# Zhengjun-Du/LC-CRF-SLAM

Measured on AMD Instinct MI355X. Metric: CRF mean-field iters/sec, higher is better.
Workload: dtype f32

## Files before the change

lc-crf-slam_amd/csrc/frame_build.h:

```cpp
#pragma once

#include "engine.h"
#include "device_math.h"
#include "fused_loop.h"

namespace lccrf {
namespace fb {

using namespace fl;

constexpr unsigned kEmptyKey = 0x80008000u;
constexpr int kHdr = 512;

struct FrameArgs {
    const float *feat[kMaxFusedK];
    float w[kMaxFusedK];
    float scale[2], inv_dp1, alpha;
    int maxN;
    const int16_t *label;
    float tbl[5];
    int n_iter, with_map;
    float relax;
    int hcap;
    int lds_total;
// ... 38 lines not shown
    const int lane = tid & 63, wave = tid >> 6;
    const int incl = wave_incl_scan(x);
    __syncthreads();
    if (lane == 63) wave_sum[wave] = incl;
    __syncthreads();
    const int ws = lane < NT / 64 ? wave_sum[lane] : 0;
    const int wincl = wave_incl_scan(ws);
    total = __builtin_amdgcn_readlane(wincl, NT / 64 - 1);
    const int wbase = __builtin_amdgcn_readlane(wincl - ws, __builtin_amdgcn_readfirstlane(wave));
    return wbase + incl - x;
}

__device__ __forceinline__ unsigned corner_key(const int16_t (&r0)[2], const uint8_t (&rk)[2], int rem)
{
    const unsigned x = (unsigned short)vertex_coord<2>(r0[0], rk[0], rem);
    const unsigned y = (unsigned short)vertex_coord<2>(r0[1], rk[1], rem);
    return x | (y << 16);
}


template <class T>
__device__ __forceinline__ const T &late_args(int offset)
{
    typedef const __attribute__((address_space(4))) unsigned char *kptr;
    kptr p = (kptr)__builtin_amdgcn_kernarg_segment_ptr();
    asm volatile("" : "+s"(p));
    return *(const T *)(p + offset);
}
constexpr int kArgOffA = (int)((sizeof(CrfDev) + alignof(FrameArgs) - 1) / alignof(FrameArgs) * alignof(FrameArgs));
static_assert(alignof(CrfDev) == 8 && alignof(FrameArgs) == 8, "the frame kernels' arguments (CrfDev, FrameArgs) as the ABI lays them out: by value, naturally aligned, in order");

constexpr int kGridMaxCells = 32768;

__device__ __forceinline__ int wave_min(int x)
{
    x = min(x, __builtin_amdgcn_update_dpp(x, x, 0x111, 0xf, 0xf, false));
    x = min(x, __builtin_amdgcn_update_dpp(x, x, 0x112, 0xf, 0xf, false));
    x = min(x, __builtin_amdgcn_update_dpp(x, x, 0x114, 0xf, 0xf, false));
    x = min(x, __builtin_amdgcn_update_dpp(x, x, 0x118, 0xf, 0xf, false));
    x = min(x, __builtin_amdgcn_update_dpp(x, x, 0x142, 0xa, 0xf, false));
    x = min(x, __builtin_amdgcn_update_dpp(x, x, 0x143, 0xc, 0xf, false));
    return x;
}

struct GridPlace {
    int row;
    int scratch_a;
    int scratch_b;
};
template <int NT, int PPT, class EmitBary>
__device__ __forceinline__ void grid_records(int tid, int N, const float2 (&ftv)[PPT], const float *scale, float inv_dp1, EmitBary emit_bary,
                                             unsigned (&pw)[PPT], unsigned (&pf)[PPT], int *box, int *fail)
{
    constexpr int D1 = kD1;
    const int Npad = (N + 3) & ~3;
    int umin = 0x7fffffff, umax = -0x7fffffff, vmin = 0x7fffffff, vmax = -0x7fffffff;
    bool bad = false;
#pragma unroll
    for (int s = 0; s < PPT; ++s) {
        const int i = tid + s * NT;
        const float2 ft = ftv[s];
        float feat[2] = {i < N ? ft.x : 0.0f, i < N ? ft.y : 0.0f};
        float b[D1];
        int r0x, r0y;
        point_record2_grid(feat, scale, inv_dp1, b, r0x, r0y, pf[s], bad);
        emit_bary(s, i, b);
        const int u = (r0x - r0y) / 3;
        if (i < Npad) {
            umin = min(umin, u); umax = max(umax, u);
            vmin = min(vmin, r0y); vmax = max(vmax, r0y);
        }
        pw[s] = ((unsigned)u & 0xffffu) | ((unsigned)r0y << 16);
    }
    const int lo_u = wave_min(umin), hi_u = wave_min(-umax), lo_v = wave_min(vmin), hi_v = wave_min(-vmax);
    if ((tid & 63) == 63) {
        atomicMin(&box[0], lo_u);
        atomicMin(&box[1], hi_u);
        atomicMin(&box[2], lo_v);
        atomicMin(&box[3], hi_v);
    }
    if (bad) *fail = 1;
}

template <int NT, int PPT, class Place, class StoreNbr>
__device__ __forceinline__ bool grid_build(unsigned char *smem, int tid, int N, const unsigned (&pw)[PPT], const unsigned (&pf)[PPT],
                                           const int *box, const int *fail, int *wave_sum, int floor_lo, int limit, Place place,
                                           StoreNbr store_nbr, int &V_out, unsigned (&pk)[PPT][kD1], int *rowmax, Instr &ins)
{
    constexpr int D1 = kD1;
    const int Npad = (N + 3) & ~3;
    unsigned cell[PPT][D1];
    const int u0 = __builtin_amdgcn_readfirstlane(box[0]) - 2, v0 = __builtin_amdgcn_readfirstlane(box[2]) - 4;
    const int Wp = -__builtin_amdgcn_readfirstlane(box[1]) - u0 + 3, Hp = -__builtin_amdgcn_readfirstlane(box[3]) - v0 + 5;
    const long cells_l = (long)Wp * Hp;
    if (__builtin_amdgcn_readfirstlane(*fail) || cells_l > kGridMaxCells) return false;
    const int cells = (int)cells_l, chunks = (cells + 7) >> 3;
    const int idmap_off = limit - chunks * 16;
    unsigned short *idmap = reinterpret_cast<unsigned short *>(smem + idmap_off);
    if (idmap_off < floor_lo + 64) return false;
    for (int u = tid; u < chunks; u += NT) reinterpret_cast<uint4 *>(idmap)[u] = make_uint4(0u, 0u, 0u, 0u);
    __syncthreads();
#pragma unroll
    for (int s = 0; s < PPT; ++s) {
        const int u = (int)(short)(pw[s] & 0xffffu), v = (int)pw[s] >> 16;
        const int c0 = (u - u0) * Hp + (v - v0);
        cell[s][0] = (unsigned)c0;
        cell[s][1] = (unsigned)(c0 + 1 + ((pf[s] & 4u) ? Hp - 3 : 0) - ((pf[s] & 1u) ? Hp : 0));
        cell[s][2] = (unsigned)(c0 + 2 + ((pf[s] & 8u) ? Hp - 3 : 0) - ((pf[s] & 2u) ? Hp : 0));
#pragma unroll
        for (int j = 0; j < D1; ++j)
            if (tid + s * NT < Npad) idmap[cell[s][j]] = (unsigned short)1;
    }
    __syncthreads();
    FL_PSTAMP();

    const int cpl = (chunks + NT - 1) / NT, c0 = tid * cpl;
    int mine = 0;
    for (int q = 0; q < cpl; ++q) {
        if (c0 + q < chunks) {
            const uint4 w = reinterpret_cast<const uint4 *>(idmap)[c0 + q];
            mine += __popc(w.x) + __popc(w.y) + __popc(w.z) + __popc(w.w);
        }
    }
    int Vk;
    int id = block_excl_scan<NT>(mine, tid, wave_sum, Vk);
    V_out = Vk;
    FL_PSTAMP();
    GridPlace gp;
    if (!place(Vk, gp)) return false;
    auto take = [&](int &o, int bytes) { const int r = o; o += (bytes + 15) & ~15; return r; };
    int vs = gp.scratch_a;
    const int vcell_off = take(vs, Vk * 2);
    const int cnt_off = take(vs, (Vk + 1) * 4);
    const int vs_d = vs;
    vs = max(vs, gp.scratch_b);
    const int E = N * D1;
    const int W = (((Npad + 31) >> 5) + 3) & ~3;
    const bool bitmap = (long)E >= 16L * Vk && vs + 5 * Vk * W + 64 <= limit;
    const int bm_off = vs, pre_off = bm_off + Vk * W * 4;
    const int list_cap = (E + 7 * Vk + 8) & ~7;
    const int list_off = vs;
    const int vs_end = bitmap ? pre_off + Vk * W / 2 : list_off + list_cap * 2;
    if (vs_d > idmap_off || vs_end > limit || Vk >= 32767 || E + 7 * Vk >= 65535) return false;
    unsigned short *vcell = reinterpret_cast<unsigned short *>(smem + vcell_off);
    unsigned *cnt = reinterpret_cast<unsigned *>(smem + cnt_off);
    unsigned *bm = reinterpret_cast<unsigned *>(smem + bm_off);
    unsigned short *pre = reinterpret_cast<unsigned short *>(smem + pre_off);
    unsigned short *list = reinterpret_cast<unsigned short *>(smem + list_off);
    for (int q = 0; q < cpl; ++q) {
        if (c0 + q < chunks) {
            uint4 w = reinterpret_cast<const uint4 *>(idmap)[c0 + q];
            unsigned h[8] = {w.x & 0xffffu, w.x >> 16, w.y & 0xffffu, w.y >> 16, w.z & 0xffffu, w.z >> 16, w.w & 0xffffu, w.w >> 16};
#pragma unroll
            for (int e = 0; e < 8; ++e) {
                if (h[e]) {
                    vcell[id] = (unsigned short)((c0 + q) * 8 + e);
                    h[e] = (unsigned)++id;
                }
            }
            w = make_uint4(h[0] | h[1] << 16, h[2] | h[3] << 16, h[4] | h[5] << 16, h[6] | h[7] << 16);
            reinterpret_cast<uint4 *>(idmap)[c0 + q] = w;
        }
    }
    for (int v = tid; v <= Vk; v += NT) cnt[v] = 0u;
    __syncthreads();
    FL_PSTAMP();

    unsigned vid[PPT][D1], arr[PPT][D1];
#pragma unroll
    for (int s = 0; s < PPT; ++s)
#pragma unroll
        for (int j = 0; j < D1; ++j) vid[s][j] = (tid + s * NT < Npad) ? (unsigned)idmap[cell[s][j]] - 1u : 0u;
#pragma unroll
    for (int s = 0; s < PPT; ++s) {
#pragma unroll
        for (int j = 0; j < D1; ++j) {
            arr[s][j] = 0u;
            if (!bitmap && tid + s * NT < N) arr[s][j] = atomicAdd(&cnt[vid[s][j]], 1u);
        }
    }
    {
        for (int t = tid; t < D1 * Vk; t += NT) {
            const int j = t >= 2 * Vk ? 2 : (t >= Vk ? 1 : 0), v = t - j * Vk;
            const int c = vcell[v], dj = j == 0 ? 1 - Hp : (j == 1 ? Hp - 2 : 1);
            store_nbr(j, v, t, (unsigned)idmap[c - dj] | ((unsigned)idmap[c + dj] << 16));
        }
    }
    __syncthreads();
    FL_PSTAMP();
    if (bitmap) {
        uint4 *b4 = reinterpret_cast<uint4 *>(bm);
        for (int u = tid; u < Vk * W / 4; u += NT) b4[u] = make_uint4(0u, 0u, 0u, 0u);
        __syncthreads();
#pragma unroll
        for (int s = 0; s < PPT; ++s) {
            const int i = tid + s * NT;
            if (i < N) {
#pragma unroll
                for (int j = 0; j < D1; ++j) atomicOr(&bm[vid[s][j] * W + (i >> 5)], 1u << (i & 31));
            }
        }
        __syncthreads();
    } else {
        uint4 *l4 = reinterpret_cast<uint4 *>(list);
        for (int u = tid; u < list_cap / 8; u += NT) l4[u] = make_uint4(0x7fff7fffu, 0x7fff7fffu, 0x7fff7fffu, 0x7fff7fffu);
    }
    FL_PSTAMP();

    if (bitmap) {
        const int lane16 = tid & 15, ng = W >> 2, gpl = (ng + 15) >> 4;
        for (int v = tid >> 4; v < Vk; v += NT / 16) {
            int pc[2] = {0, 0}, sum = 0;
#pragma unroll
            for (int u = 0; u < 2; ++u) {
                const int g = lane16 * gpl + u;
                if (u < gpl && g < ng) {
                    const uint4 b = *reinterpret_cast<const uint4 *>(bm + v * W + 4 * g);
                    pc[u] = __popc(b.x) + __popc(b.y) + __popc(b.z) + __popc(b.w);
                }
                sum += pc[u];
            }
            int incl = sum;
            incl += __builtin_amdgcn_update_dpp(0, incl, 0x111, 0xf, 0xf, false);
            incl += __builtin_amdgcn_update_dpp(0, incl, 0x112, 0xf, 0xf, false);
            incl += __builtin_amdgcn_update_dpp(0, incl, 0x114, 0xf, 0xf, false);
            incl += __builtin_amdgcn_update_dpp(0, incl, 0x118, 0xf, 0xf, false);
            int run = incl - sum;
#pragma unroll
            for (int u = 0; u < 2; ++u) {
                const int g = lane16 * gpl + u;
                if (u < gpl && g < ng) pre[v * ng + g] = (unsigned short)run;
                run += pc[u];
            }
            if (lane16 == 15) cnt[v] = (unsigned)incl;
        }
        __syncthreads();
    }
    unsigned short *row = reinterpret_cast<unsigned short *>(smem + gp.row);
    {
        const int vper = (Vk + 1 + NT - 1) / NT, v0 = tid * vper;
        unsigned sum = 0u;
        int mx = 0;
        for (int u = 0; u < vper; ++u) {
            const int v = v0 + u;
            if (v < Vk) {
                const unsigned n = cnt[v];
                sum += n | (((n + 7u) & ~7u) << 16);
                mx = max(mx, (int)n);
            }
        }
        int tot;
        unsigned run = (unsigned)block_excl_scan<NT>((int)sum, tid, wave_sum, tot);
        for (int u = 0; u < vper; ++u) {
            const int v = v0 + u;
            if (v <= Vk) {
                const unsigned n = v < Vk ? cnt[v] : 0u;
                row[v] = (unsigned short)(run & 0xffffu);
                cnt[v] = (run >> 16) | (n << 16);
                run += n | (((n + 7u) & ~7u) << 16);
            }
        }
        if (rowmax) {
#pragma unroll
            for (int o = 32; o > 0; o >>= 1) mx = max(mx, __shfl_xor(mx, o, 64));
            if ((tid & 63) == 0 && mx > 0) atomicMax(rowmax, mx);
        }
    }
    __syncthreads();
    FL_PSTAMP();

    if (!bitmap) {
#pragma unroll
        for (int s = 0; s < PPT; ++s) {
            const int i = tid + s * NT;
            if (i < N) {
#pragma unroll
                for (int j = 0; j < D1; ++j) list[(cnt[vid[s][j]] & 0xffffu) + arr[s][j]] = (unsigned short)(i * D1 + j);
            }
        }
        __syncthreads();
    }
    FL_PSTAMP();
    auto below = [](const uint4 &x, unsigned e) {
        const unsigned e2 = e | (e << 16), hi = 0x80008000u;
        return 8u - (unsigned)(__popc(((x.x | hi) - e2) & hi) + __popc(((x.y | hi) - e2) & hi) + __popc(((x.z | hi) - e2) & hi) +
                               __popc(((x.w | hi) - e2) & hi));
    };
#pragma unroll
    for (int s = 0; s < PPT; ++s) {
        const int i = tid + s * NT, ic = min(i, N - 1);
        const bool real = i < N;
#pragma unroll
        for (int j = 0; j < D1; ++j) {
            const unsigned v = vid[s][j];
            unsigned r;
            if (bitmap) {
                const uint4 bq = *reinterpret_cast<const uint4 *>(bm + v * W + ((ic >> 5) & ~3));
                const int wq = (ic >> 5) & 3;
                const unsigned low = (1u << (ic & 31)) - 1u;
                r = pre[v * (W >> 2) + (ic >> 7)] + (wq > 0 ? __popc(bq.x) : 0) + (wq > 1 ? __popc(bq.y) : 0) + (wq > 2 ? __popc(bq.z) : 0) +
                    __popc((wq == 0 ? bq.x : wq == 1 ? bq.y : wq == 2 ? bq.z : bq.w) & low);
            } else {
                const unsigned lcv = cnt[v], e = (unsigned)(i * D1 + j);
                const uint4 *lp = reinterpret_cast<const uint4 *>(list + (lcv & 0xffffu));
                r = below(lp[0], e);
                const int n8 = (int)(((lcv >> 16) + 7u) >> 3);
                for (int u = 1; u < n8; ++u) r += below(lp[u], e);
            }
            pk[s][j] = (v + 1u) | (((unsigned)row[v] + (real ? r : 0u)) << 16);
        }
    }
    FL_PSTAMP();
    __syncthreads();
    return true;
}

bool frame_lean_plausible(int NA, int K, int F);
void launch_frame_lean(const CrfDev &c, const FrameArgs &a, int NA, hipStream_t s);

}
}
```

lc-crf-slam_amd/csrc/frame_lean.hip:

```cpp
#include "frame_build.h"
#include "fused_lean.h"

#include <algorithm>
#include <type_traits>

namespace lccrf {
namespace fb {

namespace {

struct LeanHdr {
    int wave_sum[16];
    int fail;
    int box[2][4];
};
constexpr int kLeanHdrBytes = 128;
static_assert(sizeof(LeanHdr) <= kLeanHdrBytes, "header");
template <int PPT>
__global__ void __launch_bounds__(kNTSmall, 4) k_frame_lean(CrfDev c, FrameArgs a)
{
    constexpr int NT = kNTSmall, K = 2, D1 = kD1;
    constexpr bool RELOAD = PPT >= 3;
    extern __shared__ __attribute__((aligned(16))) unsigned char smem[];
    const int f = blockIdx.x, tid = threadIdx.x;
// ... 21 lines not shown
    }
    constexpr int kLds = (int)kLdsHalf;
    constexpr int hdr_off = kLds - kLeanHdrBytes;
    LeanHdr *hdr = reinterpret_cast<LeanHdr *>(smem + hdr_off);

    unsigned char *rec = a.rec + (size_t)f * kLeanRecBytes;
    PointRegs<PPT, K> pr;
    {
        int lab[PPT];
        float2 unr[PPT];
#pragma unroll
        for (int s = 0; s < PPT; ++s) {
            const int ic = min(tid + s * NT, N - 1);
            lab[s] = 0;
            unr[s] = make_float2(0.f, 0.f);
            if (a.label) lab[s] = a.label[(size_t)f * a.maxN + ic];
            else unr[s] = reinterpret_cast<const float2 *>(c.unary)[(size_t)f * c.maxN + ic];
        }
#pragma unroll
        for (int s = 0; s < PPT; ++s) {
            const int i = tid + s * NT;
            float2 un = unr[s];
            if (a.label) {
                const int t = lab[s];
                const bool known = t >= 0 && t < 2;
                un.x = !known ? a.tbl[0] : (t == 0 ? a.tbl[3] : a.tbl[2]);
                un.y = !known ? a.tbl[0] : (t == 1 ? a.tbl[4] : a.tbl[1]);
            }
            if (!RELOAD) pr.un[s] = un;
            else if (i < N) reinterpret_cast<float2 *>(rec + kLeanRecUnary)[i] = un;
        }
    }
    if (tid < 32) reinterpret_cast<float *>(smem)[tid] = 0.0f;
    if (tid < 8) hdr->box[tid >> 2][tid & 3] = 0x7fffffff;
    if (tid == 0) hdr->fail = 0;
    __syncthreads();

    size_t plan = 128;
    int V[K];
    unsigned pk[PPT][K][D1];

    unsigned pw[K][PPT], pf[K][PPT];
    {
        float2 ftv[K][PPT];
#pragma unroll
        for (int k = 0; k < K; ++k)
#pragma unroll
            for (int s = 0; s < PPT; ++s) ftv[k][s] = reinterpret_cast<const float2 *>(a.feat[k])[(size_t)f * a.maxN + min(tid + s * NT, N - 1)];
#pragma unroll
        for (int k = 0; k < K; ++k) {
            auto emit_bary = [&](int s, int i, const float (&b)[D1]) {
                if (!RELOAD) {
#pragma unroll
                    for (int j = 0; j < D1; ++j) pr.bary[s][k][j] = b[j];
                } else if (i < N) {
                    float *bo = reinterpret_cast<float *>(rec + kLeanRecBary + k * (kLeanRecPoints * D1 * 4)) + i * D1;
#pragma unroll
                    for (int j = 0; j < D1; ++j) bo[j] = b[j];
                }
            };
            grid_records<NT, PPT>(tid, N, ftv[k], a.scale, a.inv_dp1, emit_bary, pw[k], pf[k], hdr->box[k], &hdr->fail);
        }
    }
    __syncthreads();
    FL_PSTAMP();
    auto build = [&](auto kc) -> bool {
        constexpr int k = decltype(kc)::value;
        const int plan_before = (int)plan;
        int lt_nbr = 0;
        auto place = [&](int Vk, GridPlace &gp) -> bool {
            if (Vk > lean_max_v(NT) || (k == 0 && (Vk > chain_max_v(NT) || Vk > 256))) return false;
            const LeanTables lt = lean_tables(plan, Vk, k == 0);
            lt_nbr = lt.nbr;
            gp.row = lt.row;
            gp.scratch_a = k == 0 ? (int)plan : plan_before;
            gp.scratch_b = (int)plan;
            return true;
        };
        auto store_nbr = [&](int j, int v, int t, unsigned word) {
            if (k == 0) reinterpret_cast<unsigned *>(smem + lt_nbr)[t] = word;
            else reinterpret_cast<unsigned *>(rec + kLeanRecNbr)[j * (kLeanRecNbrAxis / 4) + v] = word;
        };
        unsigned pkk[PPT][D1];
        const bool ok = grid_build<NT, PPT>(smem, tid, N, pw[k], pf[k], hdr->box[k], &hdr->fail, hdr->wave_sum, plan_before, hdr_off, place,
                                            store_nbr, V[k], pkk, nullptr, ins);
#pragma unroll
        for (int s = 0; s < PPT; ++s)
#pragma unroll
            for (int j = 0; j < D1; ++j) pk[s][k][j] = pkk[s][j];
        return ok;
    };
    if (!build(std::integral_constant<int, 0>{}) || !build(std::integral_constant<int, 1>{})) {
        flag_unfit();
        return;
    }
    FL_STAMP();

    FusedLayout lay;
#pragma unroll
    for (int k = 0; k < K; ++k) V[k] = __builtin_amdgcn_readfirstlane(V[k]);
    {
        if (!layout_lean(N, K, V, kChainMinRow, &lay, NT, (size_t)kLds) || !lay.chain0) {
            flag_unfit();
            return;
        }
    }
    if (tid == 0) {
#pragma unroll
        for (int k = 0; k < K; ++k) {
            reinterpret_cast<float2 *>(smem + lay.val[k][0])[0] = make_float2(0.f, 0.f);
            reinterpret_cast<float2 *>(smem + lay.val[k][1])[0] = make_float2(0.f, 0.f);
        }
    }
    const FrameArgs &al = late_args<FrameArgs>(kArgOffA);
    const CrfDev &cl_ = late_args<CrfDev>(0);
    float wk[K], alpha[K];
    LeanSrc src;
    const __amdgpu_buffer_rsrc_t rsrc = lean_rsrc(rec, kLeanRecBytes);
#pragma unroll
    for (int k = 0; k < K; ++k) {
        wk[k] = al.w[k];
        alpha[k] = al.alpha;
        src.nbr[k] = src.bary[k] = src.norm[k] = rsrc;
        src.off_nbr[k] = kLeanRecNbr;
        src.off_bary[k] = kLeanRecBary + k * (kLeanRecPoints * D1 * 4);
        src.off_norm[k] = kLeanRecNorm + k * (kLeanRecPoints * 4);
        src.nbr_axis_bytes[k] = kLeanRecNbrAxis;
    }
    src.unary = rsrc;
    src.off_unary = kLeanRecUnary;
    __syncthreads();

    ChainLane cl = chain_setup_lean<NT>(smem, lay, V[0], tid);
    place_products_lean<PPT, K, 1, NT>(smem, lay, N, tid, pk, pr);
    FL_STAMP();

#pragma unroll
    for (int s = 0; s < PPT; ++s) pr.q[s] = make_float2(1.0f, 1.0f);
    int t = lane_id();
    mean_field_lean<PPT, K, 1, NT, RELOAD, true>(smem, lay, V, N, t, pr, cl, alpha, wk, src, 1, 0.0f, 0.0f, ins);
    __syncthreads();
    FL_STAMP();

    t = lane_id();
    if (RELOAD) {
#pragma unroll
        for (int s = 0; s < PPT; ++s) {
            typedef unsigned lean_u2 __attribute__((ext_vector_type(2)));
            const lean_u2 u = __builtin_amdgcn_raw_buffer_load_b64(src.unary, (t + s * NT) * 8, src.off_unary, 0);
            pr.un[s] = make_float2(__uint_as_float(u.x), __uint_as_float(u.y));
        }
    }
    start_inference<PPT, K, NT>(pr, N, t);
    mean_field_lean<PPT, K, 1, NT, RELOAD, false>(smem, lay, V, N, t, pr, cl, alpha, wk, src, al.n_iter, al.relax, al.omr, ins);
    t = lane_id();
    store_results<PPT, K, NT>(cl_, f, N, t, pr, al.with_map);
    if (t < K && al.V_out[t]) al.V_out[t][f] = t == 0 ? V[0] : V[K - 1];
    if (t == 0 && al.frame_status) al.frame_status[f] = 0;
    FL_STAMP();
    if (kInstr && al.timing && (int)blockIdx.x == al.timing_block && t == al.timing_lane) al.timing[63] = ins.n;
}

template <int PPT>
void launch_lean_ppt(const CrfDev &c, const FrameArgs &a, hipStream_t s)
{
    auto fn = k_frame_lean<PPT>;
    (void)hipFuncSetAttribute(reinterpret_cast<const void *>(fn), hipFuncAttributeMaxDynamicSharedMemorySize, (int)kLdsLimit);
// ... 24 lines not shown
```

lc-crf-slam_amd/csrc/fused_lean.h:

```cpp
#pragma once

#include "fused_loop.h"

#ifndef LCCRF_LEAN_SKIP
#define LCCRF_LEAN_SKIP 0
#endif
#define LEAN_SKIP(bit) ((LCCRF_LEAN_SKIP & (bit)) != 0)

namespace lccrf {
namespace fl {

constexpr int kLeanMaxRounds = 4;
__host__ __device__ constexpr int lean_rounds(int nt) { return nt >= 512 ? 3 : 4; }
__host__ __device__ constexpr int lean_max_v(int nt) { return 3 * (nt - 64); }

__host__ __device__ inline int lean_plane_floats(int NA, int V0)
{
    const int top = V0 < kChainTop ? V0 : kChainTop;
    return (NA * kD1 + 11 * top + 3 * (V0 - top) + 16 + 63) & ~63;
}

__host__ __device__ inline bool lean_chain_wanted(int NA, int V0, int row0, int nt)
{
    return row0 >= kChainMinRow && V0 <= chain_max_v(nt) && V0 <= 256 && lean_plane_floats(NA, V0) < 65535;
// ... 36 lines not shown
            L.val[k][0] = lt.val0;
            L.val[k][1] = lt.val1;
            L.nbr[k] = lt.nbr;
            L.row[k] = lt.row;
            const size_t pb = (size_t)L.Ecap[k] * 2 * sizeof(float);
            shared_prod = pb > shared_prod ? pb : shared_prod;
        }
        if (o > 65535) return false;
        L.pstart = chain0 ? take((size_t)(V[0] + 2) * sizeof(unsigned short)) : 0;
        const int p = take(shared_prod < 1024 ? 1024 : shared_prod);
        for (int k = 0; k < K; ++k) L.prod[k] = p;
        L.total = (int)o;
        if (o <= lds_limit) {
            *lay = L;
            return true;
        }
    }
    return false;
}

#define LCCRF_ASM_SEL(off, vlo, vhi, S)                                                                             \
    "v_cmp_lt_i32_e32 vcc, " #off ", %[rem]\n\tv_cndmask_b32_e32 %[" #S "], 0, %[ad], vcc\n\t"                     \
    "ds_read_b128 v[" #vlo ":" #vhi "], %[" #S "] offset:" #off "\n\t"

__device__ __forceinline__ float chain_rows_sel(unsigned addr, int bytes, unsigned trips, unsigned &keep0, unsigned &keep1)
{
    float acc = 0.0f;
    if (trips == 0) return acc;
    unsigned sa, sb;
    asm volatile(
        LCCRF_ASM_SEL(0, 96, 99, sa) LCCRF_ASM_SEL(16, 100, 103, sb)
        LCCRF_ASM_SEL(32, 104, 107, sa) LCCRF_ASM_SEL(48, 108, 111, sb)
        LCCRF_ASM_SEL(64, 112, 115, sa) LCCRF_ASM_SEL(80, 116, 119, sb)
        "1:\n\t"
        LCCRF_ASM_SEL(96, 120, 123, sa) LCCRF_ASM_SEL(112, 124, 127, sb)
        "s_waitcnt lgkmcnt(6)\n\t"
        LCCRF_ASM_ADD8(v96, v97, v98, v99, v100, v101, v102, v103)
        "v_add_u32_e32 %[ad], 0x80, %[ad]\n\t"
        "v_subrev_u32_e32 %[rem], 0x80, %[rem]\n\t"
        LCCRF_ASM_SEL(0, 96, 99, sa) LCCRF_ASM_SEL(16, 100, 103, sb)
        "s_waitcnt lgkmcnt(6)\n\t"
        LCCRF_ASM_ADD8(v104, v105, v106, v107, v108, v109, v110, v111)
        LCCRF_ASM_SEL(32, 104, 107, sa) LCCRF_ASM_SEL(48, 108, 111, sb)
        "s_waitcnt lgkmcnt(6)\n\t"
        LCCRF_ASM_ADD8(v112, v113, v114, v115, v116, v117, v118, v119)
        LCCRF_ASM_SEL(64, 112, 115, sa) LCCRF_ASM_SEL(80, 116, 119, sb)
        "s_waitcnt lgkmcnt(6)\n\t"
        LCCRF_ASM_ADD8(v120, v121, v122, v123, v124, v125, v126, v127)
        "s_sub_u32 %[n], %[n], 1\n\t"
        "s_cmp_lg_u32 %[n], 0\n\t"
        "s_cbranch_scc1 1b\n\t"
        "s_waitcnt lgkmcnt(0)\n\t"
        : [acc] "+v"(acc), [ad] "+v"(addr), [rem] "+v"(bytes), [n] "+s"(trips), [sa] "=&v"(sa), [sb] "=&v"(sb), "+v"(keep0), "+v"(keep1)
        :
        : "scc", "vcc", "memory", LCCRF_CHAIN_RING_CLOBBERS);
    return acc;
}

__device__ __forceinline__ float chain_rows_keep(unsigned addr, unsigned end, unsigned trips, unsigned &keep0, unsigned &keep1)
{
    float acc = 0.0f;
    if (trips == 0) return acc;
    const unsigned e1 = end - 32u, e2 = end - 64u, e3 = end - 96u;
    unsigned sel;
    asm volatile(LCCRF_CHAIN_ROWS_ASM
                 : [acc] "+v"(acc), [ad] "+v"(addr), [n] "+s"(trips), [sel] "=&v"(sel), "+v"(keep0), "+v"(keep1)
                 : [e0] "v"(end), [e1] "v"(e1), [e2] "v"(e2), [e3] "v"(e3)
                 : "scc", "memory", LCCRF_CHAIN_RING_CLOBBERS);
    return acc;
}

__device__ __forceinline__ float2 lds_f2(unsigned addr)
{
#if defined(__HIP_DEVICE_COMPILE__)
    typedef float lean_f2 __attribute__((ext_vector_type(2)));
    const lean_f2 v = *reinterpret_cast<const __attribute__((address_space(3))) lean_f2 *>((unsigned long)addr);
    return make_float2(v.x, v.y);
#else
    (void)addr;
    return make_float2(0.f, 0.f);
#endif
}

__device__ __forceinline__ void lds_store_f(unsigned addr, float v)
{
#if defined(__HIP_DEVICE_COMPILE__)
    *reinterpret_cast<__attribute__((address_space(3))) float *>((unsigned long)addr) = v;
#else
    (void)addr; (void)v;
#endif
}
__device__ __forceinline__ void lds_store_f2(unsigned addr, float a, float b)
{
#if defined(__HIP_DEVICE_COMPILE__)
    typedef float lean_f2 __attribute__((ext_vector_type(2)));
    lean_f2 v;
    v.x = a;
    v.y = b;
    *reinterpret_cast<__attribute__((address_space(3))) lean_f2 *>((unsigned long)addr) = v;
#else
    (void)addr; (void)a; (void)b;
#endif
}

template <int PPT, int K, int CH>
__device__ __forceinline__ void point_products_lean(const FusedLayout &lay, const PointRegs<PPT, K> &pr, int s, int k)
{
    const unsigned a0 = (pr.ix[s][k][1] >> 16) << 2, a1 = (pr.ix[s][k][2] & 0xffffu) << 2, a2 = (pr.ix[s][k][2] >> 16) << 2;
    if (chain_k<CH>(lay, k)) {
        const unsigned pb = (unsigned)lay.Ecap[k] * 4u;
        lds_store_f(a0, pr.bary[s][k][0] * pr.q[s].x);
        lds_store_f(a0 + pb, pr.bary[s][k][0] * pr.q[s].y);
        lds_store_f(a1, pr.bary[s][k][1] * pr.q[s].x);
        lds_store_f(a1 + pb, pr.bary[s][k][1] * pr.q[s].y);
        lds_store_f(a2, pr.bary[s][k][2] * pr.q[s].x);
        lds_store_f(a2 + pb, pr.bary[s][k][2] * pr.q[s].y);
    } else {
        lds_store_f2(a0, pr.bary[s][k][0] * pr.q[s].x, pr.bary[s][k][0] * pr.q[s].y);
        lds_store_f2(a1, pr.bary[s][k][1] * pr.q[s].x, pr.bary[s][k][1] * pr.q[s].y);
        lds_store_f2(a2, pr.bary[s][k][2] * pr.q[s].x, pr.bary[s][k][2] * pr.q[s].y);
    }
}

template <int PPT, int K>
__device__ __forceinline__ float2 slice_point_lean(const PointRegs<PPT, K> &pr, int s, int k, float alpha)
{
    const float2 x0 = lds_f2(pr.ix[s][k][0] & 0xffffu), x1 = lds_f2(pr.ix[s][k][0] >> 16), x2 = lds_f2(pr.ix[s][k][1] & 0xffffu);
    const float w0 = pr.bary[s][k][0] * alpha, w1 = pr.bary[s][k][1] * alpha, w2 = pr.bary[s][k][2] * alpha;
    float t0 = w0 * x0.x, t1 = w0 * x0.y;
    t0 += w1 * x1.x; t1 += w1 * x1.y;
    t0 += w2 * x2.x; t1 += w2 * x2.y;
    return make_float2(t0, t1);
}

template <int NT>
__device__ __forceinline__ ChainLane chain_setup_lean(unsigned char *smem, const FusedLayout &lay, int V0, int tid)
{
    constexpr int k = 0;
    ChainLane cl{0u, 0u};
    int *hist = reinterpret_cast<int *>(smem + lay.prod[k]);
    if (tid < 128) hist[tid] = 0;
    __syncthreads();
    const unsigned short *row = reinterpret_cast<const unsigned short *>(smem + lay.row[k]);
    unsigned short *srt = reinterpret_cast<unsigned short *>(smem + lay.prod[k]) + 256;
    unsigned short *pstart = reinterpret_cast<unsigned short *>(smem + lay.pstart);
    int key = 0;
    if (tid < V0) {
        const int len = (int)row[tid + 1] - (int)row[tid];
        key = 63 - min((len + 3) >> 4, 63);
        atomicAdd(&hist[key], 1);
    }
    __syncthreads();
    if (tid < 64) {
        const int x = hist[tid];
        int incl = x;
#pragma unroll
        for (int o = 1; o < 64; o <<= 1) {
            const int y = __shfl_up(incl, o, 64);
            if (tid >= o) incl += y;
        }
        hist[64 + tid] = incl - x;
    }
    __syncthreads();
    if (tid < V0) srt[atomicAdd(&hist[64 + key], 1)] = (unsigned short)tid;
    __syncthreads();
    if (tid < 64) {
        int sz[4], sum = 0;
#pragma unroll
        for (int u = 0; u < 4; ++u) {
            const int r = tid * 4 + u;
            sz[u] = 0;
            if (r < V0) {
                const int v = srt[r];
                const int rl = (int)row[v + 1] - (int)row[v];
                sz[u] = ((rl + 3) & ~3) + (r < kChainTop ? 8 : 0);
            }
            sum += sz[u];
        }
        int incl = sum;
#pragma unroll
        for (int o = 1; o < 64; o <<= 1) {
            const int y = __shfl_up(incl, o, 64);
            if (tid >= o) incl += y;
        }
        int base = incl - sum;
#pragma unroll
        for (int u = 0; u < 4; ++u) {
            const int r = tid * 4 + u;
            if (r < V0) pstart[srt[r]] = (unsigned short)base;
            base += sz[u];
        }
    }
    __syncthreads();
    const int l = (tid >> 6) & 1, pr = tid >> 7, ln = tid & 63;
    const int r = pr == 0 ? (chain_top_rank(ln) >= 0 ? chain_top_rank(ln) : V0) : kChainTop + ((pr - 1) << 6) + ln;
    unsigned quads = 0, addr = 0;
    if (r < V0) {
        const int v = srt[r];
        const int rl = (int)row[v + 1] - (int)row[v], len4 = (rl + 3) & ~3;
        addr = (unsigned)(lay.prod[k] + 4 * (l * lay.Ecap[k] + (int)pstart[v]));
        quads = (unsigned)(len4 >> 2);
        cl.b = quads | ((unsigned)(len4 - rl) << 13) | ((unsigned)((v + 1) * 2 + l) << 16);
    }
    unsigned m = quads;
#pragma unroll
    for (int o = 32; o > 0; o >>= 1) m = max(m, (unsigned)__shfl_xor((int)m, o));
    cl.a = addr | (m << 18);
    __syncthreads();
    return cl;
}

__device__ __forceinline__ void chain_pads_lean(unsigned char *smem, const ChainLane &cl, int tid)
{
    if (cl.b >> 16) {
        float *e = reinterpret_cast<float *>(smem + (cl.a & 0x3ffffu)) + (cl.b & 0x1fffu) * 4u;
        const unsigned npad = (cl.b >> 13) & 3u;
        for (unsigned z = 1; z <= npad; ++z) e[-(int)z] = 0.0f;
        if ((tid >> 7) == 0) {
            reinterpret_cast<float4 *>(e)[0] = make_float4(0.f, 0.f, 0.f, 0.f);
            reinterpret_cast<float4 *>(e)[1] = make_float4(0.f, 0.f, 0.f, 0.f);
        }
    }
}

template <int PPT, int K, int CH, int NT>
__device__ __forceinline__ void place_products_lean(unsigned char *smem, const FusedLayout &lay, int N, int tid,
                                                    const unsigned (&pk)[PPT][K][kD1], PointRegs<PPT, K> &pr)
{
#pragma unroll
    for (int k = 0; k < K; ++k) {
        const unsigned short *row = reinterpret_cast<const unsigned short *>(smem + lay.row[k]);
        const unsigned short *pstart = reinterpret_cast<const unsigned short *>(smem + lay.pstart);
#pragma unroll
        for (int s = 0; s < PPT; ++s) {
            const unsigned vb = (unsigned)lay.val[k][kD1 & 1];
            pr.ix[s][k][0] = (vb + 8u * (pk[s][k][0] & 0xffffu)) | ((vb + 8u * (pk[s][k][1] & 0xffffu)) << 16);
            pr.ix[s][k][1] = vb + 8u * (pk[s][k][2] & 0xffffu);
            pr.ix[s][k][2] = 0;
            if (tid + s * NT < N) {
                unsigned sl[kD1];
#pragma unroll
                for (int j = 0; j < kD1; ++j) {
                    sl[j] = pk[s][k][j] >> 16;
                    if (chain_k<CH>(lay, k)) {
                        const int v = (int)(pk[s][k][j] & 0xffffu) - 1;
                        sl[j] = (unsigned)((int)pstart[v] + ((int)(pk[s][k][j] >> 16) - (int)row[v]));
                        sl[j] = ((unsigned)lay.prod[k] >> 2) + sl[j];
                    } else {
                        sl[j] = ((unsigned)lay.prod[k] >> 2) + 2u * sl[j];
                    }
                }
                pr.ix[s][k][1] |= sl[0] << 16;
                pr.ix[s][k][2] = sl[1] | (sl[2] << 16);
            }
        }
    }
}

typedef unsigned lean_u3 __attribute__((ext_vector_type(3)));
struct LeanSrc {
    __amdgpu_buffer_rsrc_t nbr[kMaxFusedK];
    __amdgpu_buffer_rsrc_t bary[kMaxFusedK];
    __amdgpu_buffer_rsrc_t norm[kMaxFusedK];
    __amdgpu_buffer_rsrc_t unary;
    int nbr_axis_bytes[kMaxFusedK];
    int off_nbr[kMaxFusedK], off_bary[kMaxFusedK], off_norm[kMaxFusedK], off_unary;
};
constexpr int kLeanRecPoints = 4 * kNTSmall;
constexpr int kLeanRecUnary = 0;
constexpr int kLeanRecBary = kLeanRecUnary + kLeanRecPoints * 8;
constexpr int kLeanRecNorm = kLeanRecBary + kMaxFusedK * kLeanRecPoints * kD1 * 4;
constexpr int kLeanRecNbr = kLeanRecNorm + kMaxFusedK * kLeanRecPoints * 4;
constexpr int kLeanRecNbrAxis = lean_max_v(kNTSmall) * 4;
constexpr int kLeanRecBytes = (kLeanRecNbr + kD1 * kLeanRecNbrAxis + 255) & ~255;
__device__ __forceinline__ __amdgpu_buffer_rsrc_t lean_rsrc(const void *p, size_t bytes)
{
    return __builtin_amdgcn_make_buffer_rsrc(const_cast<void *>(p), 0, (int)bytes, 0x00020000);
}

template <int PPT, int K>
__device__ __forceinline__ void opaque_ids(PointRegs<PPT, K> &pr)
{
#pragma unroll
    for (int s = 0; s < PPT; ++s) {
#pragma unroll
        for (int k = 0; k < K; ++k) asm volatile("" : "+v"(pr.ix[s][k][0]), "+v"(pr.ix[s][k][1]), "+v"(pr.ix[s][k][2]));
    }
}

struct LeanPrepPlan {
    int cl_off;
    int row_off[kMaxFusedK], row_bytes[kMaxFusedK];
    int nbr_off[kMaxFusedK], nbr_bytes[kMaxFusedK];
    int total;
};
__host__ __device__ inline LeanPrepPlan lean_prep_plan(const FusedLayout &lay, int K, const int *Vcap, int nt, int ppt)
{
    LeanPrepPlan p{};
    int o = K * ppt * nt * 12;
    p.cl_off = o;
    o += nt * 8;
    for (int k = 0; k < K; ++k) {
        p.row_off[k] = o;
        p.row_bytes[k] = ((Vcap[k] + 2) * 2 + 15) & ~15;
        o += p.row_bytes[k];
        p.nbr_off[k] = o;
        p.nbr_bytes[k] = lay.nbr[k] >= 0 ? ((kD1 * Vcap[k] * 4 + 15) & ~15) : 0;
        o += p.nbr_bytes[k];
    }
    p.total = (o + 255) & ~255;
    return p;
}

template <int PPT, int K, int CH, int NT, bool RELOAD, bool NORM = false, bool PRELOADED = false>
__device__ __forceinline__ void mean_field_lean(unsigned char *smem, const FusedLayout &lay, const int (&V)[K], int N, int &t,
                                                PointRegs<PPT, K> &pr, ChainLane &cl, const float (&alpha)[K],
                                                const float (&wk)[K], const LeanSrc &src, int n_iter, float relax, float omr, Instr &ins)
{
    constexpr int D1 = kD1;
    constexpr int KF = K - 1;
    const int wave_base = __builtin_amdgcn_readfirstlane(t & ~63);
    (void)wave_base;
#define LEAN_FRESH_T()                                                                                               \
    do {                                                                                                             \
        int z_ = 0;                                                                                                  \
        asm volatile("" : "+v"(z_));                                                                                 \
        t = wave_base + (int)__builtin_amdgcn_mbcnt_hi(~0u, __builtin_amdgcn_mbcnt_lo(~0u, (unsigned)z_));          \
    } while (0)
    auto load_weights = [&]() {
        if (!RELOAD) return;
#pragma unroll
        for (int s = 0; s < PPT; ++s) {
            const int i = t + s * NT;
            if (!NORM) {
                typedef unsigned lean_u2 __attribute__((ext_vector_type(2)));
                const lean_u2 u = __builtin_amdgcn_raw_buffer_load_b64(src.unary, i * 8, src.off_unary, 0);
                pr.un[s] = make_float2(__uint_as_float(u.x), __uint_as_float(u.y));
            }
#pragma unroll
            for (int k = 0; k < K; ++k) {
                const lean_u3 b = __builtin_amdgcn_raw_buffer_load_b96(src.bary[k], i * (D1 * 4), src.off_bary[k], 0);
                pr.bary[s][k][0] = __uint_as_float(b.x);
                pr.bary[s][k][1] = __uint_as_float(b.y);
                pr.bary[s][k][2] = __uint_as_float(b.z);
                if (!NORM) pr.wn[s][k] = __uint_as_float(__builtin_amdgcn_raw_buffer_load_b32(src.norm[k], i * 4, src.off_norm[k], 0));
            }
        }
        if (NORM) return;
#pragma unroll
        for (int s = 0; s < PPT; ++s)
#pragma unroll
            for (int k = 0; k < K; ++k) pr.wn[s][k] = wk[k] * pr.wn[s][k];
    };
    auto phase_P = [&](int k) {
#pragma unroll
        for (int s = 0; s < PPT; ++s)
            if (t + s * NT < N) point_products_lean<PPT, K, CH>(lay, pr, s, k);
        if (chain_k<CH>(lay, k)) chain_pads_lean(smem, cl, t);
    };
    auto phase_S = [&](int k) {
        float *val = reinterpret_cast<float *>(smem + lay.val[k][0]);
        if (chain_k<CH>(lay, k)) {
            const int npairs = 1 + ((max(V[k] - kChainTop, 0) + 63) >> 6);
            if (__builtin_expect((t >> 7) < npairs, 1)) {
                FL_PSTAMP();
                if ((t >> 7) == 0) __builtin_amdgcn_s_setprio(3);
                asm volatile("" : "+v"(cl.a), "+v"(cl.b));
                if (__builtin_expect((cl.b >> 16) != 0, 1) && !LEAN_SKIP(2)) {
                    const unsigned row_addr = cl.a & 0x3ffffu, row_end = row_addr + (cl.b & 0x1fffu) * 16u;
                    const unsigned m = (unsigned)__builtin_amdgcn_readfirstlane((int)(cl.a >> 18));
                    const float acc = (t >> 7) == 0 ? chain_rows_keep(row_addr, row_end, (((m + 1u) >> 1) + 3u) >> 2, cl.a, cl.b)
                                                      : chain_rows_sel(row_addr, (int)((cl.b & 0x1fffu) * 16u), (m + 7u) >> 3, cl.a, cl.b);
                    val[cl.b >> 16] = acc;
                }
                LEAN_FRESH_T();
                if ((t >> 7) == 0) __builtin_amdgcn_s_setprio(0);
                FL_PSTAMP();
            }
            return;
        }
        if (LEAN_SKIP(32)) return;
        const float2 *pl = reinterpret_cast<const float2 *>(smem + lay.prod[k]);
        const float2 *zero = reinterpret_cast<const float2 *>(smem + lay.zero);
        const unsigned short *row = reinterpret_cast<const unsigned short *>(smem + lay.row[k]);
        constexpr int RS = (K == 2 && CH == 0) ? 1 : lean_rounds(NT);
        for (int base = 0; base < lean_rounds(NT); base += RS) {
            int p0[RS], pe[RS];
#pragma unroll
            for (int r = 0; r < RS; ++r) {
                const int v = t + (base + r) * NT;
                p0[r] = pe[r] = 0;
                if (v < V[k]) { p0[r] = row[v]; pe[r] = row[v + 1]; }
            }
            float2 x[RS][8];
#pragma unroll
            for (int r = 0; r < RS; ++r) {
                const unsigned base = (unsigned)lay.prod[k] + 8u * (unsigned)p0[r];
                const int n = pe[r] - p0[r];
#pragma unroll
                for (int u = 0; u < 8; ++u) x[r][u] = lds_f2(((u < n) ? base : 0u) + 8u * u);
            }
#pragma unroll
            for (int r = 0; r < RS; ++r) {
                const int v = t + (base + r) * NT;
                float a0 = 0.0f, a1 = 0.0f;
#pragma unroll
                for (int u = 0; u < 8; ++u) { a0 += x[r][u].x; a1 += x[r][u].y; }
                for (int p = p0[r] + 8; p < pe[r] && !LEAN_SKIP(16); p += 8) {
                    float2 y[8];
#pragma unroll
                    for (int u = 0; u < 8; ++u) y[u] = *((p + u < pe[r]) ? pl + p + u : zero);
#pragma unroll
                    for (int u = 0; u < 8; ++u) { a0 += y[u].x; a1 += y[u].y; }
                }
                if (v < V[k]) reinterpret_cast<float2 *>(val)[v + 1] = make_float2(a0, a1);
            }
        }
        (void)V;
    };
    constexpr int R = lean_rounds(NT);
    constexpr int OVL_K = (K == 2 && CH == 1) ? 1 : K;
    auto load_nbr = [&](unsigned (&w)[OVL_K][D1][R]) {
#pragma unroll
        for (int k = 0; k < K; ++k) {
#pragma unroll
            for (int j = 0; j < D1; ++j) {
#pragma unroll
                for (int r = 0; r < R; ++r) {
                    w[k][j][r] = 0;
                    if (!(CH == 1 && k == 0) && (r == 0 || r * NT < V[k]))
                        w[k][j][r] = __builtin_amdgcn_raw_buffer_load_b32(src.nbr[k], (t + r * NT) * 4, src.off_nbr[k] + j * src.nbr_axis_bytes[k], 0);
                }
            }
        }
    };
    auto blur_pass = [&](int j, const unsigned (&w)[OVL_K][D1][R]) {
#pragma unroll
        for (int k = 0; k < K; ++k) {
            const float2 *src_v = reinterpret_cast<const float2 *>(smem + lay.val[k][j & 1]);
            float2 *dst = reinterpret_cast<float2 *>(smem + lay.val[k][(j & 1) ^ 1]);
            const bool in_lds = CH == 1 && k == 0;
            const unsigned *lds = reinterpret_cast<const unsigned *>(smem + (in_lds ? lay.nbr[k] : 0)) + j * V[k];
#pragma unroll
            for (int r = 0; r < (in_lds ? 1 : R); ++r) {
                const int v = t + r * NT;
                if (v < V[k]) {
                    const unsigned n = in_lds ? lds[v] : w[k][j][r];
                    const float2 o = src_v[v + 1], x = src_v[n & 0xffffu], y = src_v[n >> 16];
                    float2 u;
                    u.x = o.x + 0.5f * (x.x + y.x);
                    u.y = o.y + 0.5f * (x.y + y.y);
                    dst[v + 1] = u;
                }
            }
        }
    };
    constexpr bool OVL = K == 2 && CH == 1;
    constexpr int NA0 = NT - 128, RA = 4;
    constexpr int NB = NT - 64, RB = 3;
    auto load_nbr_ovl = [&](unsigned (&wa)[RA], unsigned (&wb)[2][RB]) {
#pragma unroll
        for (int r = 0; r < RA; ++r) {
            wa[r] = 0;
            if ((r == 0 || r * NA0 < V[K - 1]) && !LEAN_SKIP(512))
                wa[r] = __builtin_amdgcn_raw_buffer_load_b32(src.nbr[K - 1], (t - 128 + r * NA0) * 4, src.off_nbr[K - 1], 0);
        }
#pragma unroll
        for (int j = 1; j < D1; ++j) {
#pragma unroll
            for (int r = 0; r < RB; ++r) {
                wb[j - 1][r] = 0;
                if ((r == 0 || r * NB < V[K - 1]) && !LEAN_SKIP(512))
                    wb[j - 1][r] = __builtin_amdgcn_raw_buffer_load_b32(src.nbr[K - 1], (t + r * NB) * 4, src.off_nbr[K - 1] + j * src.nbr_axis_bytes[K - 1], 0);
            }
        }
    };
    auto blur_vertex = [&](const float2 *src_v, float2 *dst, int v, unsigned n) {
        if (LEAN_SKIP(64)) return;
        const float2 o = src_v[v + 1], x = src_v[n & 0xffffu], y = src_v[n >> 16];
        float2 u;
        u.x = o.x + 0.5f * (x.x + y.x);
        u.y = o.y + 0.5f * (x.y + y.y);
        dst[v + 1] = u;
    };
    auto blur_big = [&](int j, int lane, int stride, int rounds, const unsigned *w) {
        constexpr int k = K - 1;
        const float2 *src_v = reinterpret_cast<const float2 *>(smem + lay.val[k][j & 1]);
        float2 *dst = reinterpret_cast<float2 *>(smem + lay.val[k][(j & 1) ^ 1]);
#pragma unroll
        for (int r = 0; r < RA; ++r) {
            if (r < rounds) {
                const int v = lane + r * stride;
                if (v < V[k]) blur_vertex(src_v, dst, v, w[r]);
            }
        }
    };
    auto blur_small = [&](int lane, int j_lo, int j_hi) {
        const unsigned *tbl = reinterpret_cast<const unsigned *>(smem + lay.nbr[0]);
#pragma unroll
        for (int j = 0; j < D1; ++j) {
            if (j < j_lo || j >= j_hi) continue;
            const float2 *src_v = reinterpret_cast<const float2 *>(smem + lay.val[0][j & 1]);
            float2 *dst = reinterpret_cast<float2 *>(smem + lay.val[0][(j & 1) ^ 1]);
            for (int v = lane; v < V[0]; v += 64) blur_vertex(src_v, dst, v, tbl[j * V[0] + v]);
            asm volatile("s_waitcnt lgkmcnt(0)" ::: "memory");
            __builtin_amdgcn_wave_barrier();
        }
    };
    auto point_update = [&](int s) {
        if constexpr (NORM) {
#pragma unroll
            for (int k = 0; k < K; ++k) {
                const float v = slice_point_lean(pr, s, k, alpha[k]).x;
                const float nrm = 1.0f / (v + 1e-20f);
                if (RELOAD) __builtin_amdgcn_raw_buffer_store_b32(__float_as_uint(nrm), src.norm[k], (t + s * NT) * 4, src.off_norm[k], 0);
                else pr.wn[s][k] = wk[k] * nrm;
            }
            return;
        }
        float nx[2] = {-pr.un[s].x, -pr.un[s].y};
#pragma unroll
        for (int k = 0; k < K; ++k) {
            const float2 t = slice_point_lean(pr, s, k, alpha[k]);
            nx[0] += pr.wn[s][k] * t.x;
            nx[1] += pr.wn[s][k] * t.y;
        }
        pr.q[s] = softmax2(nx[0], nx[1], pr.q[s], relax, omr);
    };

    if (n_iter <= 0) return;
    if (!PRELOADED) load_weights();
#pragma unroll
    for (int s = 0; s < PPT; ++s)
        if (t + s * NT < N) point_products_lean<PPT, K, CH>(lay, pr, s, KF);
    if (chain_k<CH>(lay, KF)) chain_pads_lean(smem, cl, t);
    for (int it = 0; it < n_iter; ++it) {
        LEAN_FRESH_T();
        if (RELOAD) opaque_ids(pr);
        else opaque(pr);
        unsigned w[OVL ? 1 : K][D1][R];
        unsigned wa[RA], wb[2][RB];
        if constexpr (OVL) load_nbr_ovl(wa, wb);
        else load_nbr(w);
        __syncthreads();
        FL_STAMP();
        phase_S(KF);
#pragma unroll
        for (int k = KF - 1; k >= 0; --k) {
            __syncthreads();
            opaque_ids(pr);
            phase_P(k);
            __syncthreads();
            phase_S(k);
        }
        if constexpr (OVL) {
            if (t >= 128) blur_big(0, t - 128, NA0, RA, wa);
            __syncthreads();
            FL_STAMP();
            LEAN_FRESH_T();
            if (t >= NB) blur_small(t - NB, 0, 2);
            else blur_big(1, t, NB, RB, wb[0]);
            __syncthreads();
            if (!NORM && !LEAN_SKIP(256)) load_weights();
            if (t < NB) blur_big(2, t, NB, RB, wb[1]);
            else blur_small(t - NB, 2, D1);
            __syncthreads();
        } else {
            __syncthreads();
            FL_STAMP();
            LEAN_FRESH_T();
            blur_pass(0, w);
            __syncthreads();
            blur_pass(1, w);
            __syncthreads();
            if (!NORM && !LEAN_SKIP(256)) load_weights();
            blur_pass(2, w);
            __syncthreads();
        }
        FL_STAMP();
        LEAN_FRESH_T();
        opaque_ids(pr);
        const bool more = it + 1 < n_iter;
#pragma unroll
        for (int s = 0; s < PPT; ++s) {
            if (t + s * NT < N && !LEAN_SKIP(128)) {
                point_update(s);
                if (more) point_products_lean<PPT, K, CH>(lay, pr, s, KF);
            }
        }
        FL_STAMP();
    }
}

#undef LEAN_FRESH_T

}
}
```

Baseline: 48.04 million.

## Specialize normalization pass to single channel and pad bitmap rows to avoid LDS conflicts

In the NORM pass, the lattice splat, blur and slice now handle only the first channel: stores write the barycentric weights directly, blur and slice use scalar floats, the chained splat skips odd waves, and a scalar gather replaces the float2 splat. Separately, grid_build gains a SKEW option that pads bitmap and prefix row strides to reduce LDS bank conflicts, and hoists the bitmap/list branch out of the rank loops. It is enabled for the lean frame build. Both parts trade extra code paths and LDS space for less work and better LDS access patterns.

```diff
diff --git a/lc-crf-slam_amd/csrc/frame_build.h b/lc-crf-slam_amd/csrc/frame_build.h
--- a/lc-crf-slam_amd/csrc/frame_build.h
+++ b/lc-crf-slam_amd/csrc/frame_build.h
@@ -144,7 +144,7 @@
     if (bad) *fail = 1;
 }
 
-template <int NT, int PPT, class Place, class StoreNbr>
+template <int NT, int PPT, bool SKEW = false, class Place, class StoreNbr>
 __device__ __forceinline__ bool grid_build(unsigned char *smem, int tid, int N, const unsigned (&pw)[PPT], const unsigned (&pf)[PPT],
                                            const int *box, const int *fail, int *wave_sum, int floor_lo, int limit, Place place,
                                            StoreNbr store_nbr, int &V_out, unsigned (&pk)[PPT][kD1], int *rowmax, Instr &ins)
@@ -199,10 +199,13 @@
     const int E = N * D1;
     const int W = (((Npad + 31) >> 5) + 3) & ~3;
     const bool bitmap = (long)E >= 16L * Vk && vs + 5 * Vk * W + 64 <= limit;
-    const int bm_off = vs, pre_off = bm_off + Vk * W * 4;
+    const int ng = W >> 2;
+    const bool skew = SKEW && vs + 4 * Vk * (W | 4) + 2 * Vk * (ng + ((2 - ng) & 3)) + 64 <= limit;
+    const int Ws = skew ? W | 4 : W, ps = skew ? ng + ((2 - ng) & 3) : ng;
+    const int bm_off = vs, pre_off = bm_off + Vk * Ws * 4;
     const int list_cap = (E + 7 * Vk + 8) & ~7;
     const int list_off = vs;
-    const int vs_end = bitmap ? pre_off + Vk * W / 2 : list_off + list_cap * 2;
+    const int vs_end = bitmap ? pre_off + Vk * ps * 2 : list_off + list_cap * 2;
     if (vs_d > idmap_off || vs_end > limit || Vk >= 32767 || E + 7 * Vk >= 65535) return false;
     unsigned short *vcell = reinterpret_cast<unsigned short *>(smem + vcell_off);
     unsigned *cnt = reinterpret_cast<unsigned *>(smem + cnt_off);
@@ -252,14 +255,14 @@
     FL_PSTAMP();
     if (bitmap) {
         uint4 *b4 = reinterpret_cast<uint4 *>(bm);
-        for (int u = tid; u < Vk * W / 4; u += NT) b4[u] = make_uint4(0u, 0u, 0u, 0u);
+        for (int u = tid; u < Vk * Ws / 4; u += NT) b4[u] = make_uint4(0u, 0u, 0u, 0u);
         __syncthreads();
 #pragma unroll
         for (int s = 0; s < PPT; ++s) {
             const int i = tid + s * NT;
             if (i < N) {
 #pragma unroll
-                for (int j = 0; j < D1; ++j) atomicOr(&bm[vid[s][j] * W + (i >> 5)], 1u << (i & 31));
+                for (int j = 0; j < D1; ++j) atomicOr(&bm[vid[s][j] * Ws + (i >> 5)], 1u << (i & 31));
             }
         }
         __syncthreads();
@@ -270,14 +273,14 @@
     FL_PSTAMP();
 
     if (bitmap) {
-        const int lane16 = tid & 15, ng = W >> 2, gpl = (ng + 15) >> 4;
+        const int lane16 = tid & 15, gpl = (ng + 15) >> 4;
         for (int v = tid >> 4; v < Vk; v += NT / 16) {
             int pc[2] = {0, 0}, sum = 0;
 #pragma unroll
             for (int u = 0; u < 2; ++u) {
                 const int g = lane16 * gpl + u;
                 if (u < gpl && g < ng) {
-                    const uint4 b = *reinterpret_cast<const uint4 *>(bm + v * W + 4 * g);
+                    const uint4 b = *reinterpret_cast<const uint4 *>(bm + v * Ws + 4 * g);
                     pc[u] = __popc(b.x) + __popc(b.y) + __popc(b.z) + __popc(b.w);
                 }
                 sum += pc[u];
@@ -291,7 +294,7 @@
 #pragma unroll
             for (int u = 0; u < 2; ++u) {
                 const int g = lane16 * gpl + u;
-                if (u < gpl && g < ng) pre[v * ng + g] = (unsigned short)run;
+                if (u < gpl && g < ng) pre[v * ps + g] = (unsigned short)run;
                 run += pc[u];
             }
             if (lane16 == 15) cnt[v] = (unsigned)incl;
@@ -348,29 +351,44 @@
         return 8u - (unsigned)(__popc(((x.x | hi) - e2) & hi) + __popc(((x.y | hi) - e2) & hi) + __popc(((x.z | hi) - e2) & hi) +
                                __popc(((x.w | hi) - e2) & hi));
     };
-#pragma unroll
-    for (int s = 0; s < PPT; ++s) {
-        const int i = tid + s * NT, ic = min(i, N - 1);
-        const bool real = i < N;
-#pragma unroll
-        for (int j = 0; j < D1; ++j) {
-            const unsigned v = vid[s][j];
-            unsigned r;
-            if (bitmap) {
-                const uint4 bq = *reinterpret_cast<const uint4 *>(bm + v * W + ((ic >> 5) & ~3));
-                const int wq = (ic >> 5) & 3;
-                const unsigned low = (1u << (ic & 31)) - 1u;
-                r = pre[v * (W >> 2) + (ic >> 7)] + (wq > 0 ? __popc(bq.x) : 0) + (wq > 1 ? __popc(bq.y) : 0) + (wq > 2 ? __popc(bq.z) : 0) +
-                    __popc((wq == 0 ? bq.x : wq == 1 ? bq.y : wq == 2 ? bq.z : bq.w) & low);
-            } else {
-                const unsigned lcv = cnt[v], e = (unsigned)(i * D1 + j);
-                const uint4 *lp = reinterpret_cast<const uint4 *>(list + (lcv & 0xffffu));
-                r = below(lp[0], e);
-                const int n8 = (int)(((lcv >> 16) + 7u) >> 3);
-                for (int u = 1; u < n8; ++u) r += below(lp[u], e);
-            }
-            pk[s][j] = (v + 1u) | (((unsigned)row[v] + (real ? r : 0u)) << 16);
-        }
+    auto rank_bitmap = [&](int s, int j) -> unsigned {
+        const int ic = min(tid + s * NT, N - 1);
+        const unsigned v = vid[s][j];
+        const uint4 bq = *reinterpret_cast<const uint4 *>(bm + v * Ws + ((ic >> 5) & ~3));
+        const int wq = (ic >> 5) & 3;
+        const unsigned low = (1u << (ic & 31)) - 1u;
+        return pre[v * ps + (ic >> 7)] + (wq > 0 ? __popc(bq.x) : 0) + (wq > 1 ? __popc(bq.y) : 0) + (wq > 2 ? __popc(bq.z) : 0) +
+               __popc((wq == 0 ? bq.x : wq == 1 ? bq.y : wq == 2 ? bq.z : bq.w) & low);
+    };
+    auto rank_list = [&](int s, int j) -> unsigned {
+        const unsigned v = vid[s][j], lcv = cnt[v], e = (unsigned)((tid + s * NT) * D1 + j);
+        const uint4 *lp = reinterpret_cast<const uint4 *>(list + (lcv & 0xffffu));
+        unsigned r = below(lp[0], e);
+        const int n8 = (int)(((lcv >> 16) + 7u) >> 3);
+        for (int u = 1; u < n8; ++u) r += below(lp[u], e);
+        return r;
+    };
+    auto put = [&](int s, int j, unsigned r) {
+        const unsigned v = vid[s][j];
+        pk[s][j] = (v + 1u) | (((unsigned)row[v] + (tid + s * NT < N ? r : 0u)) << 16);
+    };
+    if constexpr (SKEW) {
+        if (bitmap) {
+#pragma unroll
+            for (int s = 0; s < PPT; ++s)
+#pragma unroll
+                for (int j = 0; j < D1; ++j) put(s, j, rank_bitmap(s, j));
+        } else {
+#pragma unroll
+            for (int s = 0; s < PPT; ++s)
+#pragma unroll
+                for (int j = 0; j < D1; ++j) put(s, j, rank_list(s, j));
+        }
+    } else {
+#pragma unroll
+        for (int s = 0; s < PPT; ++s)
+#pragma unroll
+            for (int j = 0; j < D1; ++j) put(s, j, bitmap ? rank_bitmap(s, j) : rank_list(s, j));
     }
     FL_PSTAMP();
     __syncthreads();
diff --git a/lc-crf-slam_amd/csrc/frame_lean.hip b/lc-crf-slam_amd/csrc/frame_lean.hip
--- a/lc-crf-slam_amd/csrc/frame_lean.hip
+++ b/lc-crf-slam_amd/csrc/frame_lean.hip
@@ -127,7 +127,7 @@
             else reinterpret_cast<unsigned *>(rec + kLeanRecNbr)[j * (kLeanRecNbrAxis / 4) + v] = word;
         };
         unsigned pkk[PPT][D1];
-        const bool ok = grid_build<NT, PPT>(smem, tid, N, pw[k], pf[k], hdr->box[k], &hdr->fail, hdr->wave_sum, plan_before, hdr_off, place,
+        const bool ok = grid_build<NT, PPT, true>(smem, tid, N, pw[k], pf[k], hdr->box[k], &hdr->fail, hdr->wave_sum, plan_before, hdr_off, place,
                                             store_nbr, V[k], pkk, nullptr, ins);
 #pragma unroll
         for (int s = 0; s < PPT; ++s)
diff --git a/lc-crf-slam_amd/csrc/fused_lean.h b/lc-crf-slam_amd/csrc/fused_lean.h
--- a/lc-crf-slam_amd/csrc/fused_lean.h
+++ b/lc-crf-slam_amd/csrc/fused_lean.h
@@ -142,6 +142,16 @@
 #endif
 }
 
+__device__ __forceinline__ float lds_f(unsigned addr)
+{
+#if defined(__HIP_DEVICE_COMPILE__)
+    return *reinterpret_cast<const __attribute__((address_space(3))) float *>((unsigned long)addr);
+#else
+    (void)addr;
+    return 0.f;
+#endif
+}
+
 __device__ __forceinline__ void lds_store_f(unsigned addr, float v)
 {
 #if defined(__HIP_DEVICE_COMPILE__)
@@ -163,10 +173,16 @@
 #endif
 }
 
-template <int PPT, int K, int CH>
+template <int PPT, int K, int CH, bool ONE = false>
 __device__ __forceinline__ void point_products_lean(const FusedLayout &lay, const PointRegs<PPT, K> &pr, int s, int k)
 {
     const unsigned a0 = (pr.ix[s][k][1] >> 16) << 2, a1 = (pr.ix[s][k][2] & 0xffffu) << 2, a2 = (pr.ix[s][k][2] >> 16) << 2;
+    if constexpr (ONE) {
+        lds_store_f(a0, pr.bary[s][k][0]);
+        lds_store_f(a1, pr.bary[s][k][1]);
+        lds_store_f(a2, pr.bary[s][k][2]);
+        return;
+    }
     if (chain_k<CH>(lay, k)) {
         const unsigned pb = (unsigned)lay.Ecap[k] * 4u;
         lds_store_f(a0, pr.bary[s][k][0] * pr.q[s].x);
@@ -191,6 +207,17 @@
     t0 += w1 * x1.x; t1 += w1 * x1.y;
     t0 += w2 * x2.x; t1 += w2 * x2.y;
     return make_float2(t0, t1);
+}
+
+template <int PPT, int K>
+__device__ __forceinline__ float slice_point_lean_x(const PointRegs<PPT, K> &pr, int s, int k, float alpha)
+{
+    const float x0 = lds_f(pr.ix[s][k][0] & 0xffffu), x1 = lds_f(pr.ix[s][k][0] >> 16), x2 = lds_f(pr.ix[s][k][1] & 0xffffu);
+    const float w0 = pr.bary[s][k][0] * alpha, w1 = pr.bary[s][k][1] * alpha, w2 = pr.bary[s][k][2] * alpha;
+    float t0 = w0 * x0;
+    t0 += w1 * x1;
+    t0 += w2 * x2;
+    return t0;
 }
 
 template <int NT>
@@ -270,9 +297,10 @@
     return cl;
 }
 
+template <bool ONE = false>
 __device__ __forceinline__ void chain_pads_lean(unsigned char *smem, const ChainLane &cl, int tid)
 {
-    if (cl.b >> 16) {
+    if ((cl.b >> 16) && !(ONE && ((cl.b >> 16) & 1u))) {
         float *e = reinterpret_cast<float *>(smem + (cl.a & 0x3ffffu)) + (cl.b & 0x1fffu) * 4u;
         const unsigned npad = (cl.b >> 13) & 3u;
         for (unsigned z = 1; z <= npad; ++z) e[-(int)z] = 0.0f;
@@ -415,14 +443,14 @@
     auto phase_P = [&](int k) {
 #pragma unroll
         for (int s = 0; s < PPT; ++s)
-            if (t + s * NT < N) point_products_lean<PPT, K, CH>(lay, pr, s, k);
-        if (chain_k<CH>(lay, k)) chain_pads_lean(smem, cl, t);
+            if (t + s * NT < N) point_products_lean<PPT, K, CH, NORM>(lay, pr, s, k);
+        if (chain_k<CH>(lay, k)) chain_pads_lean<NORM>(smem, cl, t);
     };
     auto phase_S = [&](int k) {
         float *val = reinterpret_cast<float *>(smem + lay.val[k][0]);
         if (chain_k<CH>(lay, k)) {
             const int npairs = 1 + ((max(V[k] - kChainTop, 0) + 63) >> 6);
-            if (__builtin_expect((t >> 7) < npairs, 1)) {
+            if (__builtin_expect((t >> 7) < npairs && !(NORM && ((t >> 6) & 1)), 1)) {
                 FL_PSTAMP();
                 if ((t >> 7) == 0) __builtin_amdgcn_s_setprio(3);
                 asm volatile("" : "+v"(cl.a), "+v"(cl.b));
@@ -440,6 +468,42 @@
             return;
         }
         if (LEAN_SKIP(32)) return;
+        if constexpr (NORM) {
+            const unsigned short *row = reinterpret_cast<const unsigned short *>(smem + lay.row[k]);
+            constexpr int RS = lean_rounds(NT);
+            int p0[RS], pe[RS];
+#pragma unroll
+            for (int r = 0; r < RS; ++r) {
+                const int v = t + r * NT;
+                p0[r] = pe[r] = 0;
+                if (v < V[k]) { p0[r] = row[v]; pe[r] = row[v + 1]; }
+            }
+            float x[RS][8];
+#pragma unroll
+            for (int r = 0; r < RS; ++r) {
+                const unsigned base = (unsigned)lay.prod[k] + 8u * (unsigned)p0[r];
+                const int n = pe[r] - p0[r];
+#pragma unroll
+                for (int u = 0; u < 8; ++u) x[r][u] = lds_f(((u < n) ? base : 0u) + 8u * u);
+            }
+#pragma unroll
+            for (int r = 0; r < RS; ++r) {
+                const int v = t + r * NT;
+                float a0 = 0.0f;
+#pragma unroll
+                for (int u = 0; u < 8; ++u) a0 += x[r][u];
+                for (int p = p0[r] + 8; p < pe[r]; p += 8) {
+                    const unsigned base = (unsigned)lay.prod[k] + 8u * (unsigned)p;
+                    float y[8];
+#pragma unroll
+                    for (int u = 0; u < 8; ++u) y[u] = lds_f(((p + u < pe[r]) ? base : 0u) + 8u * u);
+#pragma unroll
+                    for (int u = 0; u < 8; ++u) a0 += y[u];
+                }
+                if (v < V[k]) val[2 * (v + 1)] = a0;
+            }
+            return;
+        }
         const float2 *pl = reinterpret_cast<const float2 *>(smem + lay.prod[k]);
         const float2 *zero = reinterpret_cast<const float2 *>(smem + lay.zero);
         const unsigned short *row = reinterpret_cast<const unsigned short *>(smem + lay.row[k]);
@@ -537,6 +601,11 @@
     };
     auto blur_vertex = [&](const float2 *src_v, float2 *dst, int v, unsigned n) {
         if (LEAN_SKIP(64)) return;
+        if constexpr (NORM) {
+            const float *s1 = reinterpret_cast<const float *>(src_v);
+            reinterpret_cast<float *>(dst)[2 * (v + 1)] = s1[2 * (v + 1)] + 0.5f * (s1[2 * (n & 0xffffu)] + s1[2 * (n >> 16)]);
+            return;
+        }
         const float2 o = src_v[v + 1], x = src_v[n & 0xffffu], y = src_v[n >> 16];
         float2 u;
         u.x = o.x + 0.5f * (x.x + y.x);
@@ -571,7 +640,7 @@
         if constexpr (NORM) {
 #pragma unroll
             for (int k = 0; k < K; ++k) {
-                const float v = slice_point_lean(pr, s, k, alpha[k]).x;
+                const float v = slice_point_lean_x(pr, s, k, alpha[k]);
                 const float nrm = 1.0f / (v + 1e-20f);
                 if (RELOAD) __builtin_amdgcn_raw_buffer_store_b32(__float_as_uint(nrm), src.norm[k], (t + s * NT) * 4, src.off_norm[k], 0);
                 else pr.wn[s][k] = wk[k] * nrm;
@@ -592,8 +661,8 @@
     if (!PRELOADED) load_weights();
 #pragma unroll
     for (int s = 0; s < PPT; ++s)
-        if (t + s * NT < N) point_products_lean<PPT, K, CH>(lay, pr, s, KF);
-    if (chain_k<CH>(lay, KF)) chain_pads_lean(smem, cl, t);
+        if (t + s * NT < N) point_products_lean<PPT, K, CH, NORM>(lay, pr, s, KF);
+    if (chain_k<CH>(lay, KF)) chain_pads_lean<NORM>(smem, cl, t);
     for (int it = 0; it < n_iter; ++it) {
         LEAN_FRESH_T();
         if (RELOAD) opaque_ids(pr);
```

Measured after the change: 48.06 million (median of 6 runs). No clear change (+0.0%).
